# mankeyboy/ASR-FeatExt-OpenCL

Hardware: AMD Instinct MI355X
Metric: audio frames/sec (16 kHz, 25 ms/10 ms, 512-pt FFT, 40 mel, 13 MFCC + delta + delta-delta) (higher is better)
Workload: dtype f32; 1 GPU; C2: 1000 synthetic 16 kHz utterances x 10 s, 25 ms/10 ms, 512-pt FFT, 40 mel, 13 MFCC + d + dd; per GPU, resident in HBM; utterances_rank0=1000, utterances_total=1000, step_pipelining=off

## Files before the change

asr-featext-opencl_amd/csrc/mfx_front512.hip:

```cpp
#include "mfx_kernels.h"

#include <hip/hip_runtime.h>

#include "mfx_dev.h"
#include "mfx_launch.h"

#include <algorithm>
#include <cstdlib>
#include "mfx_delta_dev.h"

namespace mfx {

namespace {

constexpr int kSlot = 512;
#ifndef MFX_WAVES512
#define MFX_WAVES512 16
#endif
constexpr int kWaves = MFX_WAVES512;
constexpr int kThreads = kWaves * 64;
constexpr int kMelOff = 304;
constexpr int kTabStride = 36;
constexpr int kSplitStride = 20;

constexpr int kDctSteps = 10;
constexpr int kDctRow = 12;
#ifndef MFX_DCT_QUARTERS
#define MFX_DCT_QUARTERS 1
#endif
constexpr int kDctQ = 10;
constexpr int kDctQPad = 12;
__device__ __forceinline__ int dct_q_pos(int m) { return kDctQPad * (m / kDctQ) + (m % kDctQ); }

__device__ __forceinline__ float row_partner_own0(float own, float x)
{
    int t = __builtin_amdgcn_update_dpp(0, __float_as_int(x), 0x140, 0xf, 0xf, true);
    t = __builtin_amdgcn_update_dpp(__float_as_int(own), t, 0x111, 0xf, 0xf, false);
    return __int_as_float(t);
}

__device__ __forceinline__ float row_mirror(float x)
{
    return __int_as_float(__builtin_amdgcn_update_dpp(0, __float_as_int(x), 0x140, 0xf, 0xf, true));
}

template <bool ALIGNED, int NM>
struct PcmRegs {
    uint32_t d[ALIGNED ? NM : 2 * NM];
};

template <bool ALIGNED, int NM>
__device__ __forceinline__ void pcm_issue(PcmRegs<ALIGNED, NM> &r, __amdgpu_buffer_rsrc_t rsrc, int voff)
{
#pragma unroll
    for (int m = 0; m < NM; ++m) {
        if (ALIGNED) {
            r.d[m] = __builtin_amdgcn_raw_buffer_load_b32(rsrc, voff + 64 * m, 0, 0);
        } else {
            r.d[2 * m] = __builtin_amdgcn_raw_buffer_load_b32(rsrc, voff + 64 * m, 0, 0);
            r.d[2 * m + 1] = __builtin_amdgcn_raw_buffer_load_b32(rsrc, voff + 64 * m + 4, 0, 0);
        }
    }
}

template <int NM>
__device__ __forceinline__ void pcm_issue_stuffed(PcmRegs<true, NM> &r, __amdgpu_buffer_rsrc_t rsrc, int voff, int row_bytes)
{
#pragma unroll
    for (int m = 0; m < NM; ++m) r.d[m] = (uint32_t)__builtin_amdgcn_raw_buffer_load_b16(rsrc, voff, row_bytes * m, 0);
}

#ifdef MFX_STAMPS
#define MFX_STAMP(i)                                                                   \
    do {                                                                               \
        unsigned long long t_;                                                         \
        __builtin_amdgcn_sched_barrier(0);                                             \
        asm volatile("s_memtime %0\n\ts_waitcnt lgkmcnt(0)" : "=s"(t_)::"memory");     \
        __builtin_amdgcn_sched_barrier(0);                                             \
        st_acc[i] += t_ - st_last;                                                     \
        st_last = t_;                                                                  \
    } while (0)
#else
#define MFX_STAMP(i)
#endif

template <bool ALIGNED, bool TO_SPEC, int NM, bool FUSE, bool STUFF = false, bool CH2 = false>
__global__ void __launch_bounds__(kThreads, 4) k_front512(FrontParams p)
{
    extern __shared__ __attribute__((aligned(16))) float smem[];
    const int tid = threadIdx.x;
    const int wave = __builtin_amdgcn_readfirstlane(tid >> 6);
    const int lane = tid & 63;
    const int stuff_sh = STUFF ? (p.stuff >= 8 ? 2 : p.stuff >= 4 ? 1 : 0) : 0;
    const int slot = lane >> 4, l = lane & 15, odd_slot = slot & 1;

    const int cols = p.cols;
    const int rounds = p.mel_rounds, RS = p.mel_row_stride, DS = p.dct_stride, nb_pad = p.nb_pad;
    float *s_win = smem;
    float *s_tw = s_win + 16 * kTabStride;
    float *s_split = s_tw + 16 * kTabStride;
    float *s_melw = s_split + 16 * kSplitStride;
    int *s_mmeta = (int *)(s_melw + 16 * RS);
    float *s_dct = (float *)(s_mmeta + 32 * rounds);
    const int dct_floats = !p.dct ? 0 : p.dct_mode == 1 ? 64 * kDctRow : cols * DS;
    float *s_wave = s_dct + dct_floats + wave * (4 * kSlot);
    float *xb = s_wave + slot * kSlot;
    float *s_delta = s_dct + dct_floats + (kWaves - 1) * (4 * kSlot);
    const int delta_floats = FUSE ? delta_wave_lds_floats(p.dl1, p.dl2) : 0;
    const int tail_floats = delta_floats > 4 * kSlot ? delta_floats : 4 * kSlot;
    int *s_ctr = (int *)(s_dct + dct_floats + (kWaves - 1) * (4 * kSlot) + tail_floats);
    unsigned *s_done = (unsigned *)(s_ctr + 4);
    if (tid == 0) *s_ctr = 0;
    if (FUSE)
        for (int i = tid; i < p.done_words; i += kThreads) s_done[i] = 0u;

    for (int i = tid; i < 256; i += kThreads) {
        ((float2 *)(s_win + (i >> 4) * kTabStride))[i & 15] = ((const float2 *)p.winpair)[i];
        ((float2 *)(s_tw + (i >> 4) * kTabStride))[i & 15] = ((const float2 *)p.twid_pass)[i];
    }
    for (int i = tid; i < 128; i += kThreads)
        ((float2 *)(s_split + (i & 15) * kSplitStride))[i >> 4] = ((const float2 *)p.twid_split)[i];
    if (!TO_SPEC) {
        for (int i = tid; i < 16 * RS; i += kThreads) s_melw[i] = p.mel_lane_w[i];
        for (int i = tid; i < 16 * rounds; i += kThreads) {
            s_mmeta[2 * i] = p.mel_lane_start[i];
            const int fid = p.mel_lane_fid[i];
            if (MFX_DCT_QUARTERS)
                s_mmeta[2 * i + 1] = p.dct_mode != 1 ? fid : fid < 0 ? 4 * kDctQPad : dct_q_pos(fid);
            else
                s_mmeta[2 * i + 1] = (fid < 0 && p.dct_mode == 1) ? 4 * kDctSteps : fid;
        }
        if (p.dct_mode == 1) {
            for (int i = tid; i < 64 * kDctRow; i += kThreads) {
                const int ln = i / kDctRow, j = i - ln * kDctRow, n = ln & 15;
                const int m = MFX_DCT_QUARTERS ? kDctQ * (ln >> 4) + j : 4 * j + (ln >> 4);
                s_dct[i] = (j < kDctSteps && m < p.num_banks && n < p.dct_len) ? p.dct[m * p.dct_len + n] : 0.f;
            }
        } else {
            for (int i = tid; i < dct_floats; i += kThreads) s_dct[i] = p.dct_t[i];
        }
    }
    for (int i = lane; i < 4 * kSlot; i += 64) s_wave[i] = 0.f;
    __syncthreads();

    const int chunk_base = FUSE ? p.blk_chunk_off[blockIdx.x] : 0;
    const int chunk_cnt = FUSE ? p.blk_chunk_off[blockIdx.x + 1] - chunk_base : 0;
    if (FUSE && wave == kWaves - 1) {
        __builtin_amdgcn_s_setprio(3);
        const int t_end = p.blk_tile_off[blockIdx.x + 1];
        int t = p.blk_tile_off[blockIdx.x];
        if (t >= t_end) return;
        DeltaTile T = p.tiles[t];
#ifdef MFX_DSTAMPS
        unsigned long long ds_acc[4] = {0, 0, 0, 0}, ds_last, ds_t, ds_ph[4] = {0, 0, 0, 0};
        asm volatile("s_memrealtime %0\n\ts_waitcnt lgkmcnt(0)" : "=s"(ds_last)::"memory");
        const unsigned long long ds_begin = ds_last;
#define DSTAMP(i)                                                                         \
    do {                                                                                  \
        asm volatile("s_memrealtime %0\n\ts_waitcnt lgkmcnt(0)" : "=s"(ds_t)::"memory");  \
        ds_acc[i] += ds_t - ds_last;                                                      \
        ds_last = ds_t;                                                                   \
    } while (0)
#else
#define DSTAMP(i)
#endif
        for (; t < t_end; ++t) {
            const DeltaTile nxt = p.tiles[t + 1];
            const int lo = __builtin_amdgcn_readfirstlane(T.dep_lo), hi = __builtin_amdgcn_readfirstlane(T.dep_hi);
            bool ok = false;
            for (int spins = 0; spins < (1 << 22); ++spins) {
                ok = true;
                for (int w = lo >> 5; w <= (hi >> 5); ++w) {
                    const int b0 = max(lo - 32 * w, 0), b1 = min(hi - 32 * w, 31);
                    const unsigned mask = (b1 == 31 ? 0xffffffffu : ((1u << (b1 + 1)) - 1u)) & ~((1u << b0) - 1u);
                    const unsigned v = __hip_atomic_load(&s_done[w], __ATOMIC_RELAXED, __HIP_MEMORY_SCOPE_WORKGROUP);
                    if ((v & mask) != mask) ok = false;
                }
                if (ok) break;
                __builtin_amdgcn_s_sleep(8);
            }
            if (!ok) {
                if (lane == 0 && p.err_flag) atomicExch(p.err_flag, 1);
                return;
            }
            __builtin_amdgcn_fence(__ATOMIC_ACQUIRE, "workgroup");
            DSTAMP(0);
            Segment sg;
            sg.src_row0 = sg.out_row0 = T.seg_row0;
            sg.n_out = 0;
            sg.shift = T.shift;
            sg.lo = T.lo;
            sg.hi = T.hi;
            sg.static_off = T.static_off;
            sg.pad = 0;
#ifdef MFX_DSTAMPS
            unsigned long long *php = ds_ph;
#else
            unsigned long long *php = nullptr;
#endif
            DeltaFill<64> fill;
            fill.issue(sg, T.r0, T.n_rows, p.dl1 + p.dl2, p.feat, lane);
            if (p.dl1 == 3 && p.dl2 == 3)
                delta_tile16<3, 3, 64>(sg, T.r0, T.n_rows, p.feat, p.out, p.out_pitch, cols, 3, 3, s_delta, lane, fill, 0, 0, php);
            else
                delta_tile16<0, 0, 64>(sg, T.r0, T.n_rows, p.feat, p.out, p.out_pitch, cols, p.dl1, p.dl2, s_delta, lane, fill,
                                       0, 0, php);
            DSTAMP(1);
            T = nxt;
        }
#ifdef MFX_DSTAMPS
        if (lane == 0 && p.spec) {
            unsigned long long *o = (unsigned long long *)p.spec + (size_t)blockIdx.x * 8;
            o[0] = ds_acc[0];
            o[1] = ds_acc[1];
            o[2] = ds_last - ds_begin;
            o[3] = (unsigned long long)(t_end - p.blk_tile_off[blockIdx.x]);
            for (int i = 0; i < 4; ++i) o[4 + i] = ds_ph[i];
        }
#endif
        return;
    }

#ifdef MFX_STAMPS
    unsigned long long st_acc[8] = {0, 0, 0, 0, 0, 0, 0, 0}, st_last, st_rt0;
    asm volatile("s_memrealtime %0\n\ts_waitcnt lgkmcnt(0)" : "=s"(st_rt0)::"memory");
    asm volatile("s_memtime %0\n\ts_waitcnt lgkmcnt(0)" : "=s"(st_last)::"memory");
#endif
    struct ChunkCtx {
        int64_t out_row;
        int n_live, odd0;
        __amdgpu_buffer_rsrc_t rsrc;
    };
    auto make_ctx = [&](int c) -> ChunkCtx {
        ChunkCtx x;
        const bool valid = c < p.n_chunks;
        const Chunk *chp = p.chunks + (valid ? c : 0);
        const int64_t pcm_off = chp->pcm_off;
        x.out_row = chp->out_row;
        const int n_frames = valid ? chp->n_frames : 0;
        const int64_t rows_left = p.row_limit - x.out_row;
        x.n_live = (int)(rows_left < n_frames ? (rows_left < 0 ? 0 : rows_left) : n_frames);
        const int64_t base_s = CH2 ? pcm_off * 2 : (ALIGNED && !STUFF) ? pcm_off : (pcm_off & ~(int64_t)1);
        x.odd0 = (CH2 || (ALIGNED && !STUFF)) ? 0 : (int)(pcm_off & 1);
        int64_t bytes_left = valid ? (((p.pcm_total - base_s) * 2 + 3) & ~(int64_t)3) : 0;
        if (bytes_left > 0xfffffff0ll) bytes_left = 0xfffffff0ll;
        if (bytes_left < 0) bytes_left = 0;
        const uintptr_t bp = (uintptr_t)(p.pcm + base_s);
        const uint32_t bp_lo = __builtin_amdgcn_readfirstlane((uint32_t)bp);
        const uint32_t bp_hi = __builtin_amdgcn_readfirstlane((uint32_t)(bp >> 32));
        const uint32_t nbytes = __builtin_amdgcn_readfirstlane((uint32_t)bytes_left);
        x.rsrc = __builtin_amdgcn_make_buffer_rsrc((void *)(((uintptr_t)bp_hi << 32) | bp_lo), 0, nbytes, 0x00020000);
        return x;
    };
    auto lane_off = [&](const ChunkCtx &x, int f) -> int {
        if (CH2) return (f * p.shift + (STUFF ? (l >> stuff_sh) : 2 * l)) * 4;
        if (STUFF) return (x.odd0 + f * p.shift + (l >> stuff_sh)) * 2;
        const int s = x.odd0 + f * p.shift + 2 * l;
        return ALIGNED ? s * 2 : (s & ~1) * 2;
    };
    const int block_id = xcd_block_id();
    auto next_index = [&]() -> int {
        int k = 0;
        if (lane == 0) k = __hip_atomic_fetch_add(s_ctr, 1, __ATOMIC_RELAXED, __HIP_MEMORY_SCOPE_WORKGROUP);
        return k;
    };
    auto chunk_of = [&](int k) -> int {
        if (FUSE) return k < chunk_cnt ? chunk_base + k : p.n_chunks;
        const long long c = (long long)block_id + (long long)k * gridDim.x;
        return c < p.n_chunks ? (int)c : p.n_chunks;
    };
    int v_a = next_index(), v_b = next_index(), v_nn = next_index();
    int c_cur = chunk_of(__builtin_amdgcn_readfirstlane(v_a));
    int c_nxt = chunk_of(__builtin_amdgcn_readfirstlane(v_b));
    ChunkCtx ccur = make_ctx(c_cur);
    ChunkCtx cnxt = make_ctx(c_nxt);
    constexpr bool kOneWord = STUFF || (ALIGNED && !CH2);
    PcmRegs<kOneWord, NM> cur;
    auto issue = [&](__amdgpu_buffer_rsrc_t rsrc, int voff) {
        if constexpr (CH2 && STUFF) {
#pragma unroll
            for (int m = 0; m < NM; ++m) cur.d[m] = __builtin_amdgcn_raw_buffer_load_b32(rsrc, voff, (64 >> stuff_sh) * m, 0);
        } else if constexpr (CH2) {
#pragma unroll
            for (int m = 0; m < NM; ++m) {
                const u32x2 d = __builtin_amdgcn_raw_buffer_load_b64(rsrc, voff, 128 * m, 0);
                cur.d[2 * m] = d[0];
                cur.d[2 * m + 1] = d[1];
            }
        } else if constexpr (STUFF) {
            pcm_issue_stuffed<NM>(cur, rsrc, voff, 32 >> stuff_sh);
        } else {
            pcm_issue<ALIGNED, NM>(cur, rsrc, voff);
        }
    };
    issue(ccur.rsrc, lane_off(ccur, slot));

    while (c_cur < p.n_chunks) {
        const int64_t out_row = ccur.out_row;
        const int n_live = ccur.n_live;
        const int odd0 = ccur.odd0;
        for (int f0 = 0; f0 < n_live; f0 += 4) {
            const int f = f0 + slot;
            const bool live = f < n_live;
            const bool last = f0 + 4 >= n_live;

            MFX_STAMP(0);
            float2 a[16];
            const bool odd = !ALIGNED && !STUFF && !CH2 && ((odd0 + f * p.shift) & 1);
            float4 wq[(NM + 1) / 2];
#pragma unroll
            for (int m = 0; m < (NM + 1) / 2; ++m) wq[m] = ((const float4 *)(s_win + l * kTabStride))[m];
#pragma unroll
            for (int m = 0; m < 16; ++m) {
                if (m < NM) {
                    float x0, x1 = 0.f;
                    if constexpr (CH2 && STUFF) {
                        x0 = stereo_mean(cur.d[m]);
                    } else if constexpr (CH2) {
                        x0 = stereo_mean(cur.d[2 * m]);
                        x1 = stereo_mean(cur.d[2 * m + 1]);
                    } else {
                        uint32_t d;
                        if constexpr (ALIGNED || STUFF) {
                            d = cur.d[m];
                        } else {
                            const uint32_t d0 = cur.d[2 * m], d1 = cur.d[2 * m + 1];
                            d = odd ? ((d0 >> 16) | (d1 << 16)) : d0;
                        }
                        x0 = (float)(int)(short)(d & 0xffffu);
                        x1 = (float)((int)d >> 16);
                    }
                    const float2 w = (m & 1) ? make_float2(wq[m >> 1].z, wq[m >> 1].w) : make_float2(wq[m >> 1].x, wq[m >> 1].y);
                    a[m] = STUFF ? make_float2(w.x * x0, 0.f) : make_float2(w.x * x0, w.y * x1);
                } else {
                    a[m] = make_float2(0.f, 0.f);
                }
            }

            issue(last ? cnxt.rsrc : ccur.rsrc, last ? lane_off(cnxt, slot) : lane_off(ccur, f + 4));

            MFX_STAMP(1);
            fft16(a);
            {
                float4 tq[8];
#pragma unroll
                for (int k = 0; k < 8; ++k) tq[k] = lds_read_b128((const float4 *)(s_tw + l * kTabStride) + k);
#pragma unroll
                for (int k = 0; k < 16; k += 2) {
                    const float4 t = tq[k >> 1];
                    if (k > 0) a[k] = cmul(a[k], make_float2(t.x, t.y));
                    a[k + 1] = cmul(a[k + 1], make_float2(t.z, t.w));
                }
            }

            MFX_STAMP(2);
#pragma unroll
            for (int k = 0; k < 16; ++k) ((float2 *)(xb + (k ^ odd_slot) * 32))[l ^ (k & 14)] = a[k];
            wave_sync();
#pragma unroll
            for (int j = 0; j < 8; ++j) {
                const float4 v = ((const float4 *)(xb + (l ^ odd_slot) * 32))[j ^ (l >> 1)];
                a[2 * j] = make_float2(v.x, v.y);
                a[2 * j + 1] = make_float2(v.z, v.w);
            }
            wave_sync();

            MFX_STAMP(3);
#if !defined(MFX_ABLATE) || MFX_ABLATE < 3
            fft16(a);
#endif

            MFX_STAMP(4);
            float mag_k[8], mag_p[8];
#if defined(MFX_ABLATE) && MFX_ABLATE >= 2
#pragma unroll
            for (int pp = 0; pp < 8; ++pp) {
                mag_k[pp] = a[pp].x + a[pp].y;
                mag_p[pp] = a[15 - pp].x + a[15 - pp].y;
            }
            const float mag128 = 0.f;
#else
            const float m128r = a[8].x + a[8].x, m128i = a[8].y + a[8].y;
            const float mag128 = __builtin_amdgcn_sqrtf(m128r * m128r + m128i * m128i);
            float4 csq[4];
#pragma unroll
            for (int j = 0; j < 4; ++j) csq[j] = ((const float4 *)(s_split + l * kSplitStride))[j];
#pragma unroll
            for (int pp = 0; pp < 8; ++pp) {
                const float zr = row_partner_own0(a[(16 - pp) & 15].x, a[15 - pp].x);
                const float zi = row_partner_own0(a[(16 - pp) & 15].y, a[15 - pp].y);
                const float2 cs = (pp & 1) ? make_float2(csq[pp >> 1].z, csq[pp >> 1].w) : make_float2(csq[pp >> 1].x, csq[pp >> 1].y);
                const float sr = a[pp].x + zr, si = a[pp].y - zi;
                const float dr = a[pp].x - zr, di = a[pp].y + zi;
                const float tr = cs.x * dr - cs.y * di;
                const float ti = cs.x * di + cs.y * dr;
                const float xr = sr + tr, xi = si + ti;
                const float yr = sr - tr, yi = si - ti;
                mag_k[pp] = __builtin_amdgcn_sqrtf(xr * xr + xi * xi);
                mag_p[pp] = __builtin_amdgcn_sqrtf(yr * yr + yi * yi);
            }
#endif

            MFX_STAMP(5);
            if (TO_SPEC) {
                if (live) {
                    float *dst = p.spec + (out_row + f) * (int64_t)p.spec_pitch;
#pragma unroll
                    for (int pp = 0; pp < 8; ++pp) {
                        if (!STUFF || l + 16 * pp <= (128 >> stuff_sh)) dst[l + 16 * pp] = mag_k[pp];
                        if (!STUFF) dst[256 - l - 16 * pp] = mag_p[pp];
                    }
                    if (l == 0 && (!STUFF || stuff_sh == 0)) dst[128] = mag128;
                }
            } else {
#if defined(MFX_ABLATE) && MFX_ABLATE >= 1
                {
                    float acc = mag128;
#pragma unroll
                    for (int pp = 0; pp < 8; ++pp) acc += mag_k[pp] + mag_p[pp];
                    float *dstx = p.feat + (out_row + (live ? f : 0)) * (int64_t)p.feat_pitch;
                    if (live && l < cols) dstx[l] = acc;
                    continue;
                }
#endif
                float *mg0 = xb + 32 * (slot & 1);
                {
                    float *mlo = mg0 + l, *mhi = mg0 + (144 - l);
#pragma unroll
                    for (int pp = 0; pp < 8; ++pp) mlo[16 * pp] = mag_k[pp];
#pragma unroll
                    for (int pp = 0; pp < 8; ++pp) mhi[16 * pp] = mag_p[7 - pp];
                    if (l == 0) mg0[128] = mag128;
                }
                wave_sync();

                const float *wrow = s_melw + l * RS;
                float *dst = p.feat + (out_row + f0) * (int64_t)p.feat_pitch + slot * p.feat_pitch;
                if (p.dct_mode == 1) {
                    float *lm = xb + kMelOff + 8 * slot;
                    const int2 *mmeta = (const int2 *)s_mmeta + l;
                    for (int r = 0; r < rounds; ++r) {
                        const int L = p.mel_L[r];
                        const int2 mt = *mmeta;
                        mmeta += 16;
                        const float *mg = mg0 + mt.x;
                        const int fid = mt.y;
                        float acc = 0.f;
                        for (int s = 0; s < L; s += 8) {
                            float4 w[2];
                            float2 mm[4];
#pragma unroll
                            for (int q = 0; q < 2; ++q) w[q] = *(const float4 *)(wrow + s + 4 * q);
#pragma unroll
                            for (int q = 0; q < 4; ++q) mm[q] = lds_read_b64((const float2 *)(mg + s + 2 * q));
#pragma unroll
                            for (int q = 0; q < 2; ++q) {
                                acc += w[q].x * mm[2 * q].x;
                                acc += w[q].y * mm[2 * q].y;
                                acc += w[q].z * mm[2 * q + 1].x;
                                acc += w[q].w * mm[2 * q + 1].y;
                            }
                        }
                        wrow += L;
                        lm[fid] = MFX_LOG(fmaxf(acc, 1e-30f));
                    }
                    wave_sync();
#if MFX_DCT_QUARTERS
                    const float4 *aq = (const float4 *)(s_wave + (lane & 3) * (kSlot + 8) + kMelOff + kDctQPad * slot);
                    const float4 *bq = (const float4 *)(s_dct + lane * kDctRow);
                    const float4 a0 = aq[0], a1 = aq[1], a2 = aq[2];
                    const float4 dq0 = bq[0], dq1 = bq[1], dq2 = bq[2];
                    f32x4 dacc = {0.f, 0.f, 0.f, 0.f}, dacc2 = {0.f, 0.f, 0.f, 0.f};
                    dacc = __builtin_amdgcn_mfma_f32_4x4x1f32(a0.x, dq0.x, dacc, 0, 0, 0);
                    dacc2 = __builtin_amdgcn_mfma_f32_4x4x1f32(a0.y, dq0.y, dacc2, 0, 0, 0);
                    dacc = __builtin_amdgcn_mfma_f32_4x4x1f32(a0.z, dq0.z, dacc, 0, 0, 0);
                    dacc2 = __builtin_amdgcn_mfma_f32_4x4x1f32(a0.w, dq0.w, dacc2, 0, 0, 0);
                    dacc = __builtin_amdgcn_mfma_f32_4x4x1f32(a1.x, dq1.x, dacc, 0, 0, 0);
                    dacc2 = __builtin_amdgcn_mfma_f32_4x4x1f32(a1.y, dq1.y, dacc2, 0, 0, 0);
                    dacc = __builtin_amdgcn_mfma_f32_4x4x1f32(a1.z, dq1.z, dacc, 0, 0, 0);
                    dacc2 = __builtin_amdgcn_mfma_f32_4x4x1f32(a1.w, dq1.w, dacc2, 0, 0, 0);
                    dacc = __builtin_amdgcn_mfma_f32_4x4x1f32(a2.x, dq2.x, dacc, 0, 0, 0);
                    dacc2 = __builtin_amdgcn_mfma_f32_4x4x1f32(a2.y, dq2.y, dacc2, 0, 0, 0);
                    const auto r01 = __builtin_amdgcn_permlane16_swap(__float_as_uint(dacc[0] + dacc2[0]), __float_as_uint(dacc[1] + dacc2[1]), false, false);
                    const auto r23 = __builtin_amdgcn_permlane16_swap(__float_as_uint(dacc[2] + dacc2[2]), __float_as_uint(dacc[3] + dacc2[3]), false, false);
                    const float s01 = __uint_as_float(r01[0]) + __uint_as_float(r01[1]);
                    const float s23 = __uint_as_float(r23[0]) + __uint_as_float(r23[1]);
                    const auto rr = __builtin_amdgcn_permlane32_swap(__float_as_uint(s01), __float_as_uint(s23), false, false);
                    const float outv = __uint_as_float(rr[0]) + __uint_as_float(rr[1]);
#else
                    const float *arow = s_wave + (l >> 2) * (kSlot + 8) + kMelOff + slot;
                    const float4 *bq = (const float4 *)(s_dct + lane * kDctRow);
                    const float4 dq0 = bq[0], dq1 = bq[1], dq2 = bq[2];
                    const float dctb[12] = {dq0.x, dq0.y, dq0.z, dq0.w, dq1.x, dq1.y, dq1.z, dq1.w, dq2.x, dq2.y, dq2.z, dq2.w};
                    f32x4 dacc = {0.f, 0.f, 0.f, 0.f}, dacc2 = {0.f, 0.f, 0.f, 0.f};
#pragma unroll
                    for (int j = 0; j < kDctSteps; j += 2) {
                        dacc = __builtin_amdgcn_mfma_f32_16x16x4f32(arow[4 * j], dctb[j], dacc, 0, 0, 0);
                        dacc2 = __builtin_amdgcn_mfma_f32_16x16x4f32(arow[4 * j + 4], dctb[j + 1], dacc2, 0, 0, 0);
                    }
                    const float outv = dacc[0] + dacc2[0];
#endif
                    if (live && (l < cols || p.feat_pitch == 16)) dst[l] = outv;
                } else {
                    float *melbuf = xb + kMelOff;
                    const int2 *mmeta = (const int2 *)s_mmeta + l;
                    for (int r = 0; r < rounds; ++r) {
                        const int L = p.mel_L[r];
                        const int2 mt = *mmeta;
                        mmeta += 16;
                        const float *mg = mg0 + mt.x;
                        const int fid = mt.y;
                        float acc = 0.f;
                        for (int s = 0; s < L; s += 4) {
                            const float4 w = *(const float4 *)(wrow + s);
                            const float2 m0 = *(const float2 *)(mg + s);
                            const float2 m1 = *(const float2 *)(mg + s + 2);
                            acc += w.x * m0.x;
                            acc += w.y * m0.y;
                            acc += w.z * m1.x;
                            acc += w.w * m1.y;
                        }
                        wrow += L;
                        if (fid >= 0) melbuf[fid] = MFX_LOG(fmaxf(acc, 1e-30f));
                    }
                    wave_sync();
                    for (int c0 = 0; c0 < cols; c0 += 16) {
                        const int cc = c0 + l;
                        const bool act = cc < cols;
                        float acc;
                        if (p.dct) {
                            const float *dm = s_dct + (act ? cc : 0) * DS;
                            acc = 0.f;
                            for (int m = 0; m < nb_pad; m += 4) {
                                const float4 mv = *(const float4 *)(melbuf + m);
                                const float4 dv = *(const float4 *)(dm + m);
                                acc += mv.x * dv.x;
                                acc += mv.y * dv.y;
                                acc += mv.z * dv.z;
                                acc += mv.w * dv.w;
                            }
                        } else {
                            acc = melbuf[act ? cc : 0];
                        }
                        if (live && act) dst[cc] = acc;
                    }
                }
                wave_sync();
            }
            MFX_STAMP(6);
        }
        if (n_live <= 0) issue(cnxt.rsrc, lane_off(cnxt, slot));
        if (FUSE) {
            __builtin_amdgcn_fence(__ATOMIC_RELEASE, "workgroup");
            const int kk = c_cur - chunk_base;
            if (lane == 0)
                __hip_atomic_fetch_or(&s_done[kk >> 5], 1u << (kk & 31), __ATOMIC_RELAXED, __HIP_MEMORY_SCOPE_WORKGROUP);
        }
        c_cur = c_nxt;
        ccur = cnxt;
        asm volatile("" : "+v"(v_nn));
        c_nxt = chunk_of(__builtin_amdgcn_readfirstlane(v_nn));
        cnxt = make_ctx(c_nxt);
        v_nn = next_index();
    }
#ifdef MFX_STAMPS
    if (lane == 0 && p.spec) {
        unsigned long long *o = (unsigned long long *)p.spec + (size_t)(blockIdx.x * kWaves + wave) * 8;
        unsigned long long st_rt1;
        asm volatile("s_memrealtime %0\n\ts_waitcnt lgkmcnt(0)" : "=s"(st_rt1)::"memory");
        st_acc[7] = st_rt1 - st_rt0;
        for (int i = 0; i < 8; ++i) o[i] = st_acc[i];
    }
#endif
}

constexpr int kSlotL = 544;
constexpr int kOddOffL = 264;
constexpr int kTrOffL = 272;
constexpr int kMelOffL = 0;
constexpr int kTabStrideO = 68;
constexpr int kDctStepsL = 20;
constexpr int kDctRowL = 20;

template <bool ALIGNED, int NM, int WAVES>
__global__ void __launch_bounds__(WAVES * 64, WAVES / 4) k_front1024(FrontParams p)
{
    extern __shared__ __attribute__((aligned(16))) float smem[];
    const int tid = threadIdx.x;
    const int wave = __builtin_amdgcn_readfirstlane(tid >> 6);
    const int lane = tid & 63;
    const int slot = lane >> 4, l = lane & 15;
    const int cols = p.cols, rounds = p.mel_rounds, RS = p.mel_row_stride;

    float *s_win = smem;
    float *s_winO = s_win + 16 * kTabStride;
    float *s_tw = s_winO + 16 * kTabStrideO;
    float *s_splitE = s_tw + 16 * kTabStride;
    float *s_splitO = s_splitE + 16 * kSplitStride;
    float *s_melw = s_splitO + 16 * kSplitStride;
    int *s_mmeta = (int *)(s_melw + 16 * RS);
    float *s_dct = (float *)(s_mmeta + 32 * rounds);
    float *s_wave = s_dct + 64 * kDctRowL + wave * (4 * kSlotL);
    float *xb = s_wave + slot * kSlotL;
    int *s_ctr = (int *)(s_dct + 64 * kDctRowL + WAVES * (4 * kSlotL));
    if (tid == 0) *s_ctr = 0;

    for (int i = tid; i < 256; i += WAVES * 64) {
        ((float2 *)(s_win + (i >> 4) * kTabStride))[i & 15] = ((const float2 *)p.winpair)[i];
        ((float4 *)(s_winO + (i >> 4) * kTabStrideO))[i & 15] = ((const float4 *)p.win1024o)[i];
        ((float2 *)(s_tw + (i >> 4) * kTabStride))[i & 15] = ((const float2 *)p.twid_pass)[i];
    }
    for (int i = tid; i < 128; i += WAVES * 64) {
        ((float2 *)(s_splitE + (i & 15) * kSplitStride))[i >> 4] = ((const float2 *)p.twid_split)[2 * i];
        ((float2 *)(s_splitO + (i & 15) * kSplitStride))[i >> 4] = ((const float2 *)p.twid_split)[2 * i + 1];
    }
    for (int i = tid; i < 16 * RS; i += WAVES * 64) s_melw[i] = p.mel_lane_w[i];
    for (int i = tid; i < 16 * rounds; i += WAVES * 64) {
        s_mmeta[2 * i] = p.mel_lane_start[i] >> 1;
        const int fid = p.mel_lane_fid[i];
        s_mmeta[2 * i + 1] = fid < 0 ? 4 * kDctStepsL : fid;
    }
    for (int i = tid; i < 64 * kDctRowL; i += WAVES * 64) {
        const int ln = i / kDctRowL, j = i - ln * kDctRowL, n = ln & 15;
        const int m = MFX_DCT_QUARTERS ? kDctStepsL * (ln >> 4) + j : 4 * j + (ln >> 4);
        s_dct[i] = (p.dct && m < p.num_banks && n < p.dct_len) ? p.dct[m * p.dct_len + n] : 0.f;
    }
    for (int i = lane; i < 4 * kSlotL; i += 64) s_wave[i] = 0.f;
    __syncthreads();

    struct ChunkCtx {
        int64_t out_row;
        int n_live, odd0;
        __amdgpu_buffer_rsrc_t rsrc;
    };
    auto make_ctx = [&](int c) -> ChunkCtx {
        ChunkCtx x;
        const bool valid = c < p.n_chunks;
        const Chunk *chp = p.chunks + (valid ? c : 0);
        const int64_t pcm_off = chp->pcm_off;
        x.out_row = chp->out_row;
        const int n_frames = valid ? chp->n_frames : 0;
        const int64_t rows_left = p.row_limit - x.out_row;
        x.n_live = (int)(rows_left < n_frames ? (rows_left < 0 ? 0 : rows_left) : n_frames);
        const int64_t base_s = ALIGNED ? pcm_off : (pcm_off & ~(int64_t)1);
        x.odd0 = ALIGNED ? 0 : (int)(pcm_off & 1);
        int64_t bytes_left = valid ? (((p.pcm_total - base_s) * 2 + 3) & ~(int64_t)3) : 0;
        if (bytes_left > 0xfffffff0ll) bytes_left = 0xfffffff0ll;
        if (bytes_left < 0) bytes_left = 0;
        const uintptr_t bp = (uintptr_t)(p.pcm + base_s);
        const uint32_t bp_lo = __builtin_amdgcn_readfirstlane((uint32_t)bp);
        const uint32_t bp_hi = __builtin_amdgcn_readfirstlane((uint32_t)(bp >> 32));
        const uint32_t nbytes = __builtin_amdgcn_readfirstlane((uint32_t)bytes_left);
        x.rsrc = __builtin_amdgcn_make_buffer_rsrc((void *)(((uintptr_t)bp_hi << 32) | bp_lo), 0, nbytes, 0x00020000);
        return x;
    };
    auto lane_off = [&](const ChunkCtx &x, int f) -> int {
        const int s = x.odd0 + f * p.shift + 2 * l;
        return ALIGNED ? s * 2 : (s & ~1) * 2;
    };
    const int block_id = xcd_block_id();
    auto next_index = [&]() -> int {
        int k = 0;
        if (lane == 0) k = __hip_atomic_fetch_add(s_ctr, 1, __ATOMIC_RELAXED, __HIP_MEMORY_SCOPE_WORKGROUP);
        return k;
    };
    auto chunk_of = [&](int k) -> int {
        const long long c = (long long)block_id + (long long)k * gridDim.x;
        return c < p.n_chunks ? (int)c : p.n_chunks;
    };
    int v_a = next_index(), v_b = next_index(), v_nn = next_index();
    int c_cur = chunk_of(__builtin_amdgcn_readfirstlane(v_a));
    int c_nxt = chunk_of(__builtin_amdgcn_readfirstlane(v_b));
    ChunkCtx ccur = make_ctx(c_cur);
    ChunkCtx cnxt = make_ctx(c_nxt);
    PcmRegs<ALIGNED, NM> cur;
    pcm_issue<ALIGNED, NM>(cur, ccur.rsrc, lane_off(ccur, slot));

    while (c_cur < p.n_chunks) {
        const int64_t out_row = ccur.out_row;
        const int n_live = ccur.n_live;
        const int odd0 = ccur.odd0;
        for (int f0 = 0; f0 < n_live; f0 += 4) {
            const int f = f0 + slot;
            const bool live = f < n_live;
            const bool last = f0 + 4 >= n_live;
            const bool odd = !ALIGNED && ((odd0 + f * p.shift) & 1);
            uint32_t dd[ALIGNED ? 1 : NM];
            if (!ALIGNED) {
#pragma unroll
                for (int m = 0; m < NM; ++m) {
                    const uint32_t d0 = cur.d[2 * m], d1 = cur.d[2 * m + 1];
                    dd[m] = odd ? __builtin_amdgcn_alignbit(d1, d0, 16) : d0;
                }
                pcm_issue<ALIGNED, NM>(cur, last ? cnxt.rsrc : ccur.rsrc, last ? lane_off(cnxt, slot) : lane_off(ccur, f + 4));
            }
            auto pair_of = [&](int m, float &x0, float &x1, bool fresh) {
                uint32_t d = ALIGNED ? cur.d[m] : dd[m];
                if (fresh) asm volatile("" : "+v"(d));
                x0 = (float)(int)(short)(d & 0xffffu);
                x1 = (float)((int)d >> 16);
            };
            auto fft256_head = [&](float2(&a)[16]) {
                fft16(a);
                float4 tq[8];
#pragma unroll
                for (int k = 0; k < 8; ++k) tq[k] = lds_read_b128((const float4 *)(s_tw + l * kTabStride) + k);
#pragma unroll
                for (int k = 0; k < 16; k += 2) {
                    const float4 t = tq[k >> 1];
                    if (k > 0) a[k] = cmul(a[k], make_float2(t.x, t.y));
                    a[k + 1] = cmul(a[k + 1], make_float2(t.z, t.w));
                }
            };

            constexpr bool FULL = NM > 16;
            static_assert(!FULL || ALIGNED, "windows longer than 512 samples: aligned frames only");
            auto folded = [&](int m, bool want_sum, bool fresh) -> float2 {
                uint32_t dA = cur.d[m], dB = (m + 16 < NM) ? cur.d[(m + 16 < NM) ? m + 16 : 0] : 0u;
                if (fresh) asm volatile("" : "+v"(dA), "+v"(dB));
                const float2 tA = ((const float2 *)(s_winO + l * kTabStrideO))[m];
                float2 r = make_float2(tA.x * (float)(int)(short)(dA & 0xffffu), tA.y * (float)((int)dA >> 16));
                if (m + 16 < NM) {
                    const float2 tB = ((const float2 *)(s_winO + l * kTabStrideO))[m + 16];
                    const float2 pB = make_float2(tB.x * (float)(int)(short)(dB & 0xffffu), tB.y * (float)((int)dB >> 16));
                    r = want_sum ? make_float2(r.x + pB.x, r.y + pB.y) : make_float2(r.x - pB.x, r.y - pB.y);
                }
                return r;
            };

            {
                float2 a[16];
                constexpr int NW = FULL ? 1 : (NM + 1) / 2;
                float4 wq[NW];
                if (!FULL) {
#pragma unroll
                    for (int m = 0; m < NW; ++m) wq[m] = ((const float4 *)(s_win + l * kTabStride))[m];
                }
#pragma unroll
                for (int m = 0; m < 16; ++m) {
                    if (FULL) {
                        a[m] = folded(m, true, false);
                    } else if (m < NM) {
                        float x0, x1;
                        pair_of(m, x0, x1, false);
                        const float2 w = (m & 1) ? make_float2(wq[m >> 1].z, wq[m >> 1].w) : make_float2(wq[m >> 1].x, wq[m >> 1].y);
                        a[m] = make_float2(w.x * x0, w.y * x1);
                    } else {
                        a[m] = make_float2(0.f, 0.f);
                    }
                }
                fft256_head(a);
#pragma unroll
                for (int k = 0; k < 16; ++k) ((float2 *)(xb + k * 32))[l ^ (k & 14)] = a[k];
                wave_sync();
#pragma unroll
                for (int j = 0; j < 8; ++j) {
                    const float4 v = ((const float4 *)(xb + l * 32))[j ^ (l >> 1)];
                    a[2 * j] = make_float2(v.x, v.y);
                    a[2 * j + 1] = make_float2(v.z, v.w);
                }
                wave_sync();
                fft16(a);
                const float m128r = a[8].x + a[8].x, m128i = a[8].y + a[8].y;
                if (l == 0) xb[128] = __builtin_amdgcn_sqrtf(m128r * m128r + m128i * m128i);
                float4 csq[4];
#pragma unroll
                for (int j = 0; j < 4; ++j) csq[j] = ((const float4 *)(s_splitE + l * kSplitStride))[j];
                float *elo = xb + l, *ehi = xb + (144 - l);
#pragma unroll
                for (int pp = 0; pp < 8; ++pp) {
                    const float zr = row_partner_own0(a[(16 - pp) & 15].x, a[15 - pp].x);
                    const float zi = row_partner_own0(a[(16 - pp) & 15].y, a[15 - pp].y);
                    const float2 cs = (pp & 1) ? make_float2(csq[pp >> 1].z, csq[pp >> 1].w) : make_float2(csq[pp >> 1].x, csq[pp >> 1].y);
                    const float sr = a[pp].x + zr, si = a[pp].y - zi;
                    const float dr = a[pp].x - zr, di = a[pp].y + zi;
                    const float tr = cs.x * dr - cs.y * di;
                    const float ti = cs.x * di + cs.y * dr;
                    const float xr = sr + tr, xi = si + ti;
                    const float yr = sr - tr, yi = si - ti;
                    elo[16 * pp] = __builtin_amdgcn_sqrtf(xr * xr + xi * xi);
                    ehi[16 * (7 - pp)] = __builtin_amdgcn_sqrtf(yr * yr + yi * yi);
                }
            }

            {
                float2 a[16];
#pragma unroll
                for (int m = 0; m < 16; ++m) {
                    if (FULL) {
                        a[m] = cmul(folded(m, false, true), ((const float2 *)(s_win + l * kTabStride))[m]);
                    } else if (m < NM) {
                        float x0, x1;
                        pair_of(m, x0, x1, true);
                        const float4 t = ((const float4 *)(s_winO + l * kTabStrideO))[m];
                        a[m] = make_float2(t.x * x0 + t.y * x1, t.z * x0 + t.w * x1);
                    } else {
                        a[m] = make_float2(0.f, 0.f);
                    }
                }
                if (ALIGNED) pcm_issue<ALIGNED, NM>(cur, last ? cnxt.rsrc : ccur.rsrc, last ? lane_off(cnxt, slot) : lane_off(ccur, f + 4));
                fft256_head(a);
                float *xt = xb + kTrOffL;
                const float4 *xrow = (const float4 *)(xt + l * 16);
#pragma unroll
                for (int k = 0; k < 16; ++k) xt[k * 16 + (l ^ (4 * (k >> 2)))] = a[k].x;
                wave_sync();
#pragma unroll
                for (int j = 0; j < 4; ++j) {
                    const float4 v = xrow[j ^ (l >> 2)];
                    a[4 * j].x = v.x;
                    a[4 * j + 1].x = v.y;
                    a[4 * j + 2].x = v.z;
                    a[4 * j + 3].x = v.w;
                }
                wave_sync();
#pragma unroll
                for (int k = 0; k < 16; ++k) xt[k * 16 + (l ^ (4 * (k >> 2)))] = a[k].y;
                wave_sync();
#pragma unroll
                for (int j = 0; j < 4; ++j) {
                    const float4 v = xrow[j ^ (l >> 2)];
                    a[4 * j].y = v.x;
                    a[4 * j + 1].y = v.y;
                    a[4 * j + 2].y = v.z;
                    a[4 * j + 3].y = v.w;
                }
                wave_sync();
                fft16(a);
                float4 csq[4];
#pragma unroll
                for (int j = 0; j < 4; ++j) csq[j] = ((const float4 *)(s_splitO + l * kSplitStride))[j];
                float *olo = xb + kOddOffL + l, *ohi = xb + kOddOffL + (143 - l);
#pragma unroll
                for (int pp = 0; pp < 8; ++pp) {
                    const float zr = row_mirror(a[15 - pp].x);
                    const float zi = row_mirror(a[15 - pp].y);
                    const float2 cs = (pp & 1) ? make_float2(csq[pp >> 1].z, csq[pp >> 1].w) : make_float2(csq[pp >> 1].x, csq[pp >> 1].y);
                    const float sr = a[pp].x + zr, si = a[pp].y - zi;
                    const float dr = a[pp].x - zr, di = a[pp].y + zi;
                    const float tr = cs.x * dr - cs.y * di;
                    const float ti = cs.x * di + cs.y * dr;
                    const float xr = sr + tr, xi = si + ti;
                    const float yr = sr - tr, yi = si - ti;
                    olo[16 * pp] = __builtin_amdgcn_sqrtf(xr * xr + xi * xi);
                    ohi[16 * (7 - pp)] = __builtin_amdgcn_sqrtf(yr * yr + yi * yi);
                }
            }
            wave_sync();

            const float *wrow = s_melw + l * RS;
            float *dst = p.feat + (out_row + f0) * (int64_t)p.feat_pitch + slot * p.feat_pitch;
            float *lm = xb + kMelOffL + 8 * slot;
            const int2 *mmeta = (const int2 *)s_mmeta + l;
            float le[kDctStepsL / 4];
#pragma unroll
            for (int r = 0; r < kDctStepsL / 4; ++r) {
                le[r] = 0.f;
                if (r < rounds) {
                    const int L = p.mel_L[r];
                    const int first = mmeta[16 * r].x;
                    const float *me = xb + first, *mo = xb + kOddOffL + first;
                    float acc = 0.f;
                    for (int s = 0; s < L; s += 8) {
                        float4 w[2];
                        float2 e[2], o[2];
#pragma unroll
                        for (int q = 0; q < 2; ++q) w[q] = *(const float4 *)(wrow + s + 4 * q);
#pragma unroll
                        for (int q = 0; q < 2; ++q) {
                            e[q] = lds_read_b64((const float2 *)(me + (s >> 1) + 2 * q));
                            o[q] = lds_read_b64((const float2 *)(mo + (s >> 1) + 2 * q));
                        }
#pragma unroll
                        for (int q = 0; q < 2; ++q) {
                            acc += w[q].x * e[q].x;
                            acc += w[q].y * o[q].x;
                            acc += w[q].z * e[q].y;
                            acc += w[q].w * o[q].y;
                        }
                    }
                    wrow += L;
                    le[r] = MFX_LOG(fmaxf(acc, 1e-30f));
                }
            }
            wave_sync();
#pragma unroll
            for (int r = 0; r < kDctStepsL / 4; ++r)
                if (r < rounds) lm[mmeta[16 * r].y] = le[r];
            wave_sync();
            if (!p.dct) {
                if (live)
                    for (int cc = l; cc < cols; cc += 16) dst[cc] = lm[cc];
            } else
            {
#if MFX_DCT_QUARTERS
                const float4 *aq = (const float4 *)(s_wave + (lane & 3) * (kSlotL + 8) + kMelOffL + kDctStepsL * slot);
                const float4 *bq = (const float4 *)(s_dct + lane * kDctRowL);
                f32x4 dacc = {0.f, 0.f, 0.f, 0.f}, dacc2 = {0.f, 0.f, 0.f, 0.f};
                float4 av[kDctStepsL / 4], bv[kDctStepsL / 4];
#pragma unroll
                for (int j = 0; j < kDctStepsL / 4; ++j) {
                    av[j] = aq[j];
                    bv[j] = bq[j];
                }
#pragma unroll
                for (int j = 0; j < kDctStepsL / 4; ++j) {
                    dacc = __builtin_amdgcn_mfma_f32_4x4x1f32(av[j].x, bv[j].x, dacc, 0, 0, 0);
                    dacc2 = __builtin_amdgcn_mfma_f32_4x4x1f32(av[j].y, bv[j].y, dacc2, 0, 0, 0);
                    dacc = __builtin_amdgcn_mfma_f32_4x4x1f32(av[j].z, bv[j].z, dacc, 0, 0, 0);
                    dacc2 = __builtin_amdgcn_mfma_f32_4x4x1f32(av[j].w, bv[j].w, dacc2, 0, 0, 0);
                }
                const auto r01 = __builtin_amdgcn_permlane16_swap(__float_as_uint(dacc[0] + dacc2[0]), __float_as_uint(dacc[1] + dacc2[1]), false, false);
                const auto r23 = __builtin_amdgcn_permlane16_swap(__float_as_uint(dacc[2] + dacc2[2]), __float_as_uint(dacc[3] + dacc2[3]), false, false);
                const float s01 = __uint_as_float(r01[0]) + __uint_as_float(r01[1]);
                const float s23 = __uint_as_float(r23[0]) + __uint_as_float(r23[1]);
                const auto rr = __builtin_amdgcn_permlane32_swap(__float_as_uint(s01), __float_as_uint(s23), false, false);
                const float outv = __uint_as_float(rr[0]) + __uint_as_float(rr[1]);
#else
                const float *arow = s_wave + (l >> 2) * (kSlotL + 8) + kMelOffL + slot;
                const float4 *bq = (const float4 *)(s_dct + lane * kDctRowL);
                float dctb[kDctStepsL];
#pragma unroll
                for (int j = 0; j < kDctStepsL / 4; ++j) {
                    const float4 t = bq[j];
                    dctb[4 * j] = t.x;
                    dctb[4 * j + 1] = t.y;
                    dctb[4 * j + 2] = t.z;
                    dctb[4 * j + 3] = t.w;
                }
                f32x4 dacc = {0.f, 0.f, 0.f, 0.f}, dacc2 = {0.f, 0.f, 0.f, 0.f};
#pragma unroll
                for (int j = 0; j < kDctStepsL; j += 2) {
                    dacc = __builtin_amdgcn_mfma_f32_16x16x4f32(arow[4 * j], dctb[j], dacc, 0, 0, 0);
                    dacc2 = __builtin_amdgcn_mfma_f32_16x16x4f32(arow[4 * j + 4], dctb[j + 1], dacc2, 0, 0, 0);
                }
                const float outv = dacc[0] + dacc2[0];
#endif
                if (live && (l < cols || p.feat_pitch == 16)) dst[l] = outv;
            }
            wave_sync();
        }
        if (n_live <= 0) pcm_issue<ALIGNED, NM>(cur, cnxt.rsrc, lane_off(cnxt, slot));
        c_cur = c_nxt;
        ccur = cnxt;
        asm volatile("" : "+v"(v_nn));
        c_nxt = chunk_of(__builtin_amdgcn_readfirstlane(v_nn));
        cnxt = make_ctx(c_nxt);
        v_nn = next_index();
    }
}

}

size_t front512_lds_bytes(const FrontParams &p)
{
    size_t f = 2 * 16 * kTabStride + 16 * kSplitStride;
    f += (size_t)16 * p.mel_row_stride;
    f += (size_t)32 * p.mel_rounds;
    f += !p.dct ? 0 : p.dct_mode == 1 ? (size_t)64 * kDctRow : (size_t)p.cols * p.dct_stride;
    f += kWaves * 4 * kSlot;
    f += 4;
    return f * sizeof(float);
}

size_t front512_delta_lds_bytes(const FrontParams &p)
{
    const size_t delta_floats = (size_t)delta_wave_lds_floats(p.dl1, p.dl2);
    size_t f = front512_lds_bytes(p) / sizeof(float);
    if (delta_floats > (size_t)4 * kSlot) f += delta_floats - 4 * kSlot;
    f += (size_t)p.done_words;
    return f * sizeof(float);
}

namespace {

template <bool A, int NM>
hipError_t launch512_delta(const FrontParams &p, hipStream_t stream)
{
    const size_t lds = front512_delta_lds_bytes(p);
    if (hipError_t e = allow_dynamic_lds((const void *)k_front512<A, false, NM, true>, lds); e != hipSuccess) return e;
    hipLaunchKernelGGL((k_front512<A, false, NM, true>), dim3(p.n_blocks), dim3(kThreads), lds, stream, p);
    return hipGetLastError();
}

template <bool A, bool S, int NM, bool STUFF = false, bool CH2 = false>
hipError_t launch512(const FrontParams &p_in, hipStream_t stream)
{
    FrontParams p = p_in;
    if (S) {
        p.mel_rounds = 0;
        p.mel_row_stride = 0;
        p.dct = nullptr;
        p.dct_mode = 0;
    }
    const size_t lds = front512_lds_bytes(p);
    if (hipError_t e = allow_dynamic_lds((const void *)k_front512<A, S, NM, false, STUFF, CH2>, lds); e != hipSuccess) return e;
    const int cap = num_cus() * (32 / kWaves) / 2;
    int blocks = p.n_chunks < cap ? p.n_chunks : cap;
    if (blocks < 1) blocks = 1;
    hipLaunchKernelGGL((k_front512<A, S, NM, false, STUFF, CH2>), dim3(blocks), dim3(kThreads), lds, stream, p);
    return hipGetLastError();
}

}

size_t front1024_lds_bytes(const FrontParams &p, int waves)
{
    size_t f = 2 * 16 * kTabStride + 16 * kTabStrideO + 2 * 16 * kSplitStride;
    f += (size_t)16 * p.mel_row_stride + (size_t)32 * p.mel_rounds;
    f += (size_t)64 * kDctRowL;
    f += (size_t)waves * 4 * kSlotL + 4;
    return f * sizeof(float);
}

bool front1024_supported(int fft_size, int window_size, int num_banks, int cols, int channels, int ceps_len)
{
    return fft_size == 1024 && window_size > 0 && window_size <= 1024 && channels <= 1 && num_banks >= 1 &&
           num_banks <= 4 * kDctStepsL && (ceps_len > 0 ? cols <= 16 : cols == num_banks);
}

namespace {
template <bool A, int NM, int WAVES>
hipError_t launch1024(const FrontParams &p, hipStream_t stream)
{
    const size_t lds = front1024_lds_bytes(p, WAVES);
    if (hipError_t e = allow_dynamic_lds((const void *)k_front1024<A, NM, WAVES>, lds); e != hipSuccess) return e;
    int blocks = (p.n_chunks + WAVES - 1) / WAVES;
    if (blocks > num_cus()) blocks = num_cus();
    if (blocks < 1) blocks = 1;
    hipLaunchKernelGGL((k_front1024<A, NM, WAVES>), dim3(blocks), dim3(WAVES * 64), lds, stream, p);
    return hipGetLastError();
}
}

int front1024_waves(const FrontParams &p, bool aligned, int nm16, int max_waves)
{
    return max_waves >= 16 && aligned && nm16 <= 16 && front1024_lds_bytes(p, 16) <= (size_t)160 * 1024 ? 16 : 12;
}

hipError_t launch_front1024(const FrontParams &p, bool aligned, int nm16, hipStream_t stream, int max_waves)
{
    if (p.n_chunks <= 0) return hipSuccess;
    if (nm16 > 16) {
        if (!aligned) return hipErrorInvalidValue;
        return nm16 <= 24 ? launch1024<true, 24, 12>(p, stream) : launch1024<true, 32, 12>(p, stream);
    }
    const bool nm13 = nm16 <= 13;
    if (front1024_waves(p, aligned, nm16, max_waves) == 16) return nm13 ? launch1024<true, 13, 16>(p, stream) : launch1024<true, 16, 16>(p, stream);
    if (aligned) return nm13 ? launch1024<true, 13, 12>(p, stream) : launch1024<true, 16, 12>(p, stream);
    return nm13 ? launch1024<false, 13, 12>(p, stream) : launch1024<false, 16, 12>(p, stream);
}

bool front512_supported(int fft_size, int window_size, int num_banks, int cols, int channels)
{
    return (fft_size == 512 || fft_size == 256 || fft_size == 128 || fft_size == 64) && window_size <= fft_size && window_size > 0 && channels <= 2 && num_banks >= 1 &&
           num_banks <= 128 && cols <= 128;
}

const char *front512_kernel_name(bool to_spectrum, bool aligned, int nm16)
{
    (void)to_spectrum;
    (void)aligned;
    (void)nm16;
    return "k_front512";
}

hipError_t launch_front512(const FrontParams &p, bool to_spectrum, bool aligned, int nm16, hipStream_t stream)
{
    if (p.n_chunks <= 0) return hipSuccess;
    const bool nm13 = nm16 <= 13;
    if (p.channels == 2) {
        if (p.stuff) {
            if (to_spectrum) return nm13 ? launch512<true, true, 13, true, true>(p, stream) : launch512<true, true, 16, true, true>(p, stream);
            return nm13 ? launch512<true, false, 13, true, true>(p, stream) : launch512<true, false, 16, true, true>(p, stream);
        }
        if (to_spectrum) return nm13 ? launch512<true, true, 13, false, true>(p, stream) : launch512<true, true, 16, false, true>(p, stream);
        return nm13 ? launch512<true, false, 13, false, true>(p, stream) : launch512<true, false, 16, false, true>(p, stream);
    }
    if (p.stuff) {
        if (to_spectrum) return nm13 ? launch512<true, true, 13, true>(p, stream) : launch512<true, true, 16, true>(p, stream);
        return nm13 ? launch512<true, false, 13, true>(p, stream) : launch512<true, false, 16, true>(p, stream);
    }
    if (to_spectrum) {
        if (aligned) return nm13 ? launch512<true, true, 13>(p, stream) : launch512<true, true, 16>(p, stream);
        return nm13 ? launch512<false, true, 13>(p, stream) : launch512<false, true, 16>(p, stream);
    }
    if (aligned) return nm13 ? launch512<true, false, 13>(p, stream) : launch512<true, false, 16>(p, stream);
    return nm13 ? launch512<false, false, 13>(p, stream) : launch512<false, false, 16>(p, stream);
}

hipError_t launch_front512_delta(const FrontParams &p, bool aligned, int nm16, hipStream_t stream)
{
    if (p.n_chunks <= 0 || p.n_blocks <= 0) return hipSuccess;
    const bool nm13 = nm16 <= 13;
    if (aligned) return nm13 ? launch512_delta<true, 13>(p, stream) : launch512_delta<true, 16>(p, stream);
    return nm13 ? launch512_delta<false, 13>(p, stream) : launch512_delta<false, 16>(p, stream);
}

}
```

Baseline: 2.847 billion frames/s.

## Overlap LDS table staging with first PCM load and skip atomic chunk claims

The constant tables (window, twiddles, mel weights, DCT) are now loaded from global memory into registers up front and written to LDS later. In the non-fused path this happens after the first PCM buffer load is issued, so table-fetch latency overlaps the first audio fetch. The initial three chunk indices are assigned statically per wave instead of through LDS atomics, and the counter starts at 3*kWaves to match. This costs extra registers per thread, and the DCT load uses inline 24-bit mad indexing. Timestamp instrumentation is added under MFX_STAMPS and does not run by default.

```diff
diff --git a/asr-featext-opencl_amd/csrc/mfx_front512.hip b/asr-featext-opencl_amd/csrc/mfx_front512.hip
--- a/asr-featext-opencl_amd/csrc/mfx_front512.hip
+++ b/asr-featext-opencl_amd/csrc/mfx_front512.hip
@@ -110,38 +110,85 @@
     const int tail_floats = delta_floats > 4 * kSlot ? delta_floats : 4 * kSlot;
     int *s_ctr = (int *)(s_dct + dct_floats + (kWaves - 1) * (4 * kSlot) + tail_floats);
     unsigned *s_done = (unsigned *)(s_ctr + 4);
-    if (tid == 0) *s_ctr = 0;
+    if (tid == 0) *s_ctr = FUSE ? 0 : 3 * kWaves;
+#ifdef MFX_STAMPS
+    unsigned long long *const st_blk = (unsigned long long *)p.spec + (size_t)gridDim.x * kWaves * 8 + (size_t)blockIdx.x * 4;
+    if (tid == 0 && p.spec) {
+        unsigned long long t_;
+        unsigned xcc_;
+        asm volatile("s_memrealtime %0\n\ts_waitcnt lgkmcnt(0)" : "=s"(t_)::"memory");
+        asm volatile("s_getreg_b32 %0, hwreg(HW_REG_XCC_ID)" : "=s"(xcc_));
+        st_blk[0] = t_;
+        st_blk[2] = xcc_ & 15u;
+        st_blk[3] = (unsigned long long)xcd_block_id();
+    }
+#endif
     if (FUSE)
         for (int i = tid; i < p.done_words; i += kThreads) s_done[i] = 0u;
 
-    for (int i = tid; i < 256; i += kThreads) {
-        ((float2 *)(s_win + (i >> 4) * kTabStride))[i & 15] = ((const float2 *)p.winpair)[i];
-        ((float2 *)(s_tw + (i >> 4) * kTabStride))[i & 15] = ((const float2 *)p.twid_pass)[i];
-    }
-    for (int i = tid; i < 128; i += kThreads)
-        ((float2 *)(s_split + (i & 15) * kSplitStride))[i >> 4] = ((const float2 *)p.twid_split)[i];
-    if (!TO_SPEC) {
-        for (int i = tid; i < 16 * RS; i += kThreads) s_melw[i] = p.mel_lane_w[i];
-        for (int i = tid; i < 16 * rounds; i += kThreads) {
-            s_mmeta[2 * i] = p.mel_lane_start[i];
-            const int fid = p.mel_lane_fid[i];
-            if (MFX_DCT_QUARTERS)
-                s_mmeta[2 * i + 1] = p.dct_mode != 1 ? fid : fid < 0 ? 4 * kDctQPad : dct_q_pos(fid);
-            else
-                s_mmeta[2 * i + 1] = (fid < 0 && p.dct_mode == 1) ? 4 * kDctSteps : fid;
-        }
+    static_assert(kThreads >= 256, "one table word per thread");
+    constexpr int kMelTrip = 4, kDctTrip = (64 * kDctRow + kThreads - 1) / kThreads;
+    float g_melw[kMelTrip], g_dct[kDctTrip];
+    bool g_dct_ok[kDctTrip];
+    int g_start = 0, g_fid = 0;
+    const float2 g_win = ((const float2 *)p.winpair)[tid & 255];
+    const float2 g_tw = ((const float2 *)p.twid_pass)[tid & 255];
+    const float2 g_split = ((const float2 *)p.twid_split)[tid & 127];
+    if (!TO_SPEC && rounds > 0 && RS > 0) {
+#pragma unroll
+        for (int q = 0; q < kMelTrip; ++q) g_melw[q] = p.mel_lane_w[min(tid + q * kThreads, 16 * RS - 1)];
+        g_start = p.mel_lane_start[min(tid, 16 * rounds - 1)];
+        g_fid = p.mel_lane_fid[min(tid, 16 * rounds - 1)];
         if (p.dct_mode == 1) {
-            for (int i = tid; i < 64 * kDctRow; i += kThreads) {
+#pragma unroll
+            for (int q = 0; q < kDctTrip; ++q) {
+                const int i = tid + q * kThreads;
                 const int ln = i / kDctRow, j = i - ln * kDctRow, n = ln & 15;
                 const int m = MFX_DCT_QUARTERS ? kDctQ * (ln >> 4) + j : 4 * j + (ln >> 4);
-                s_dct[i] = (j < kDctSteps && m < p.num_banks && n < p.dct_len) ? p.dct[m * p.dct_len + n] : 0.f;
-            }
-        } else {
-            for (int i = tid; i < dct_floats; i += kThreads) s_dct[i] = p.dct_t[i];
+                g_dct_ok[q] = i < 64 * kDctRow && j < kDctSteps && m < p.num_banks && n < p.dct_len;
+                unsigned idx;
+                asm("v_mad_u32_u24 %0, %1, %2, %3" : "=v"(idx) : "v"(m), "v"(p.dct_len), "v"(n));
+                g_dct[q] = p.dct[g_dct_ok[q] ? idx : 0u];
+            }
         }
     }
-    for (int i = lane; i < 4 * kSlot; i += 64) s_wave[i] = 0.f;
-    __syncthreads();
+    auto stage_store = [&]() {
+        if (tid < 256) {
+            ((float2 *)(s_win + (tid >> 4) * kTabStride))[tid & 15] = g_win;
+            ((float2 *)(s_tw + (tid >> 4) * kTabStride))[tid & 15] = g_tw;
+        }
+        if (tid < 128) ((float2 *)(s_split + (tid & 15) * kSplitStride))[tid >> 4] = g_split;
+        if (!TO_SPEC) {
+#pragma unroll
+            for (int q = 0; q < kMelTrip; ++q) {
+                const int i = tid + q * kThreads;
+                if (i < 16 * RS) s_melw[i] = g_melw[q];
+            }
+            for (int i = tid + kMelTrip * kThreads; i < 16 * RS; i += kThreads) s_melw[i] = p.mel_lane_w[i];
+            if (tid < 16 * rounds) {
+                s_mmeta[2 * tid] = g_start;
+                if (MFX_DCT_QUARTERS)
+                    s_mmeta[2 * tid + 1] = p.dct_mode != 1 ? g_fid : g_fid < 0 ? 4 * kDctQPad : dct_q_pos(g_fid);
+                else
+                    s_mmeta[2 * tid + 1] = (g_fid < 0 && p.dct_mode == 1) ? 4 * kDctSteps : g_fid;
+            }
+            if (p.dct_mode == 1) {
+#pragma unroll
+                for (int q = 0; q < kDctTrip; ++q) {
+                    const int i = tid + q * kThreads;
+                    asm volatile("" : "+v"(g_dct[q]));
+                    if (i < 64 * kDctRow) s_dct[i] = g_dct_ok[q] ? g_dct[q] : 0.f;
+                }
+            } else {
+                for (int i = tid; i < dct_floats; i += kThreads) s_dct[i] = p.dct_t[i];
+            }
+        }
+        for (int i = lane; i < 4 * kSlot; i += 64) s_wave[i] = 0.f;
+    };
+    if constexpr (FUSE) {
+        stage_store();
+        __syncthreads();
+    }
 
     const int chunk_base = FUSE ? p.blk_chunk_off[blockIdx.x] : 0;
     const int chunk_cnt = FUSE ? p.blk_chunk_off[blockIdx.x + 1] - chunk_base : 0;
@@ -222,8 +269,9 @@
     }
 
 #ifdef MFX_STAMPS
-    unsigned long long st_acc[8] = {0, 0, 0, 0, 0, 0, 0, 0}, st_last, st_rt0;
+    unsigned long long st_acc[8] = {0, 0, 0, 0, 0, 0, 0, 0}, st_last, st_rt0, st_first = 0;
     asm volatile("s_memrealtime %0\n\ts_waitcnt lgkmcnt(0)" : "=s"(st_rt0)::"memory");
+    if (FUSE && tid == 0 && p.spec) st_blk[1] = st_rt0;
     asm volatile("s_memtime %0\n\ts_waitcnt lgkmcnt(0)" : "=s"(st_last)::"memory");
 #endif
     struct ChunkCtx {
@@ -269,7 +317,12 @@
         const long long c = (long long)block_id + (long long)k * gridDim.x;
         return c < p.n_chunks ? (int)c : p.n_chunks;
     };
-    int v_a = next_index(), v_b = next_index(), v_nn = next_index();
+    int v_a, v_b, v_nn;
+    if constexpr (FUSE) {
+        v_a = next_index(), v_b = next_index(), v_nn = next_index();
+    } else {
+        v_a = wave, v_b = wave + kWaves, v_nn = wave + 2 * kWaves;
+    }
     int c_cur = chunk_of(__builtin_amdgcn_readfirstlane(v_a));
     int c_nxt = chunk_of(__builtin_amdgcn_readfirstlane(v_b));
     ChunkCtx ccur = make_ctx(c_cur);
@@ -294,6 +347,17 @@
         }
     };
     issue(ccur.rsrc, lane_off(ccur, slot));
+    if constexpr (!FUSE) {
+        stage_store();
+        __syncthreads();
+#ifdef MFX_STAMPS
+        if (tid == 0 && p.spec) {
+            unsigned long long t_;
+            asm volatile("s_memrealtime %0\n\ts_waitcnt lgkmcnt(0)" : "=s"(t_)::"memory");
+            st_blk[1] = t_;
+        }
+#endif
+    }
 
     while (c_cur < p.n_chunks) {
         const int64_t out_row = ccur.out_row;
@@ -340,6 +404,10 @@
             issue(last ? cnxt.rsrc : ccur.rsrc, last ? lane_off(cnxt, slot) : lane_off(ccur, f + 4));
 
             MFX_STAMP(1);
+#ifdef MFX_STAMPS
+            if (st_first == 0)
+                asm volatile("s_memrealtime %0\n\ts_waitcnt lgkmcnt(0)" : "=s"(st_first)::"memory");
+#endif
             fft16(a);
             {
                 float4 tq[8];
@@ -570,6 +638,9 @@
         asm volatile("s_memrealtime %0\n\ts_waitcnt lgkmcnt(0)" : "=s"(st_rt1)::"memory");
         st_acc[7] = st_rt1 - st_rt0;
         for (int i = 0; i < 8; ++i) o[i] = st_acc[i];
+        unsigned long long *w = (unsigned long long *)p.spec + (size_t)gridDim.x * (kWaves * 8 + 4) + (size_t)(blockIdx.x * kWaves + wave) * 2;
+        w[0] = st_rt1;
+        w[1] = st_first;
     }
 #endif
 }
```

Result: no change. 2.862 billion frames/s (median of 2 runs) (+0.5%).
